# KexinZhangResearch/PhysDock

Hardware: AMD Instinct MI355X
Metric: poses/sec (whole node) at crop_size=256, atom_crop_size=2048 (higher is better)
Workload: dtype f32 (fp16x2-split operands x3 MFMA / bf16x3-split x6 MFMA, fp32 accumulate)

## Files before the change

physdock_amd/csrc/gemm_f16.hip:

```cpp
#include <stdlib.h>
#include <type_traits>
#define PD_EPILOGUE_Y2 1
#include "gemm_tile_common.h"

namespace {

typedef _Float16 f16x8 __attribute__((ext_vector_type(8)));
typedef _Float16 f16x4 __attribute__((ext_vector_type(4)));
typedef unsigned u32x2 __attribute__((ext_vector_type(2)));

constexpr int F16_MIN_TILES = 256, F16_MIN_TILES_SMALL = 160, F16_MIN_TILES_SMALL_LONGK = 96;
#ifdef PD_LAB
__device__ unsigned long long* g_f16_trace = nullptr;
#define PD_TRACE_F16_PTR g_f16_trace
#else
#define PD_TRACE_F16_PTR ((unsigned long long*)nullptr)
#endif
constexpr int NPARTS = 2;
constexpr int PITCH = 24;
constexpr int PITCH2 = 40;

template <int BM_, int BN_, int WM_, int NWAVES_, bool DW_>
struct FTile {
    static constexpr int BM = BM_, BN = BN_, WM = WM_, WN = NWAVES_ / WM_, NT = 64 * NWAVES_;
    static constexpr int TM = BM / (32 * WM), TN = BN / (32 * WN);
    static constexpr bool DW = DW_;
    static constexpr int STAGE = DW ? NPARTS * BM * PITCH2 : NPARTS * (BM + BN) * PITCH;
    static constexpr int LDS_BYTES = 2 * STAGE * 2;
    static constexpr int BLOCKS_PER_CU = NWAVES_ == 8 ? 2 : 4;
    static constexpr int WAVES_PER_SIMD = NWAVES_ * BLOCKS_PER_CU / 4;
    static constexpr int GRID = 256 * BLOCKS_PER_CU;
};

__device__ __forceinline__ void lds_barrier() {
    asm volatile("" ::: "memory");
    __builtin_amdgcn_s_waitcnt(0xc07f);
    __builtin_amdgcn_s_barrier();
    asm volatile("" ::: "memory");
}

__device__ __forceinline__ void split4h(const f32x4& v, f16x4& h, f16x4& l) {
    const pd_parts2 p0 = pd_split2h(v[0], v[1]), p1 = pd_split2h(v[2], v[3]);
    h = __builtin_bit_cast(f16x4, (u32x2){p0.h, p1.h});
    l = __builtin_bit_cast(f16x4, (u32x2){p0.l, p1.l});
}

template <int PRO, int EPI, class TL>
__global__ __launch_bounds__(TL::NT) __attribute__((amdgpu_waves_per_eu(TL::WAVES_PER_SIMD, TL::WAVES_PER_SIMD)))
void gemm_f16_kernel(const pd_gemm_args p) {
    constexpr int BM = TL::BM, BN = TL::BN, TM = TL::TM, TN = TL::TN;
    constexpr int XSLOTS = TL::GRID / 8;
    constexpr int SNT = TL::NT;
    constexpr int TPR_A = SNT / BM;
    constexpr int CPH_A = 4 / TPR_A;
    constexpr int TPR_W = SNT / BN;
    constexpr int NW = 4 / TPR_W;
    constexpr bool DW = TL::DW;
    extern __shared__ __attribute__((aligned(16))) _Float16 lds[];
    const int tid = threadIdx.x, lane = tid & 63;
    const int wave = __builtin_amdgcn_readfirstlane(tid >> 6);
    const int wm = wave / TL::WN, wn = wave % TL::WN;
    const int l31 = lane & 31, hh = lane >> 5;
    const int nMb = p.M / BM, nNb = p.N / BN;
    const int ntiles = nMb * nNb;
    const int nk = (p.K + 31) / 32;
    const int nks = 2 * nk;
    const f16x8* __restrict__ W2 = reinterpret_cast<const f16x8*>(p.W2);
    const long long wpart = (long long)((p.N + 31) / 32) * nks * 64;
    auto w2_chunk = [&](int part, int n, int kchunk) {
        return W2 + part * wpart + ((long long)(n >> 5) * nks + (kchunk >> 1)) * 64 + (kchunk & 1) * 32 + (n & 31);
    };
    const float a_s = pd_pow2_scale(*p.a_amax);
    const float inv_a_s = 1.0f / a_s;

    auto sA = [&](int s, int part) { return lds + s * TL::STAGE + part * BM * PITCH; };
    auto sW = [&](int s, int part) { return lds + s * TL::STAGE + NPARTS * BM * PITCH + part * BN * PITCH; };

    const int a_row = tid / TPR_A, a_q = tid % TPR_A;
    const int w_row = tid / TPR_W, w_q = tid % TPR_W;
    constexpr bool AS = PRO == 3;
    constexpr int CPA = 4 / TPR_A;
    const _Float16* __restrict__ A2 = reinterpret_cast<const _Float16*>(p.A2);
    const long long apart = (long long)p.M * (nk * 32);
    f16x8 ra2[NPARTS][AS ? CPA : 1];
    f32x4 ra[2][CPH_A];
    f16x8 rw[NPARTS][NW];

    auto gload = [&](int bm0, int bn0, int k0) {
        const int r = bm0 + a_row;
        if constexpr (AS) {
            const _Float16* ap2 = A2 + (long long)r * (nk * 32) + k0 + 8 * a_q;
#pragma unroll
            for (int part = 0; part < NPARTS; ++part)
#pragma unroll
                for (int i = 0; i < CPA; ++i) ra2[part][i] = *reinterpret_cast<const f16x8*>(ap2 + part * apart + 8 * TPR_A * i);
        }
        const float* ap = p.A + (long long)r * p.lda + k0;
#pragma unroll
        for (int h = 0; h < (AS ? 0 : 2); ++h)
#pragma unroll
            for (int i = 0; i < CPH_A; ++i) {
                int kc = 16 * h + 4 * (a_q + TPR_A * i);
                kc = k0 + kc < p.K ? kc : 0;
                ra[h][i] = *reinterpret_cast<const f32x4*>(ap + kc);
            }
        if constexpr (!DW) {
#pragma unroll
            for (int part = 0; part < NPARTS; ++part)
#pragma unroll
                for (int i = 0; i < NW; ++i)
                    rw[part][i] = *w2_chunk(part, bn0 + w_row, (k0 >> 3) + (NW == 2 ? w_q + 2 * i : w_q));
        }
    };
    f16x8 wf[2][TN][NPARTS];
    auto wfrag = [&](int buf, int bn0, int ks) {
#pragma unroll
        for (int j = 0; j < TN; ++j) {
            const f16x8* base = W2 + ((long long)((bn0 + wn * (32 * TN) + j * 32) >> 5) * nks + ks) * 64 + lane;
#pragma unroll
            for (int part = 0; part < NPARTS; ++part) wf[buf][j][part] = base[part * wpart];
        }
    };

    f32x16 acc[TM][TN];
    const bool grouped = gridDim.x == TL::GRID && nMb >= 8;
    TileOrder ord;
    ord.init(nMb, nNb, grouped ? blockIdx.x & 7 : 0, grouped ? 8 : 1, XSLOTS);
    const int t_step = grouped ? XSLOTS : gridDim.x;
    const int t_end = grouped ? ord.ntiles : ntiles;
    int tile = grouped ? blockIdx.x >> 3 : blockIdx.x;
    if (tile >= t_end) return;
    auto coords = [&](int t, int& bm0, int& bn0) {
        int mb, nb;
        if (grouped) ord.get(t, mb, nb);
        else { mb = t % nMb; nb = t / nMb; }
        bm0 = mb * BM; bn0 = nb * BN;
    };
    int bm0, bn0;
    coords(tile, bm0, bn0);
    gload(bm0, bn0, 0);
    if constexpr (DW) { wfrag(0, bn0, 0); wfrag(1, bn0, 1); }

    for (; tile < t_end; tile += t_step) {
        const int n0 = bn0 + wn * (32 * TN) + l31;
        float c0[TN], c1[TN], cs[TN];
        const int gate_row = bm0 + wm * (32 * TM);
#pragma unroll
        for (int j = 0; j < TN; ++j) {
            c0[j] = p.bias ? p.bias[n0 + 32 * j] : 0.f;
            c1[j] = 1.f;
            cs[j] = p.w_inv[n0 + 32 * j] * inv_a_s;
            if constexpr (EPI == EPI_HN) c1[j] = p.hn_w[((n0 + 32 * j) / p.hn_split) * 32 + l31];
            if constexpr (EPI == EPI_GATERES)
                c1[j] = p.mul ? p.mul[(long long)(gate_row / p.mul_rows_per_group) * p.mul_gstride + n0 + 32 * j] : 1.f;
        }
        float st_mean = 0.f, st_rstd = 1.f;
        int grp_off = 0;
        if constexpr (PRO != 0 && !AS) {
            const int m = bm0 + a_row;
            st_mean = p.stats[2 * (long long)m];
            st_rstd = p.stats[2 * (long long)m + 1];
            if constexpr (PRO == 2) grp_off = (m / p.pro_rows_per_group) * p.pro_gstride;
        }
        auto prep = [&](f32x4 v, int kc, f16x4& ph, f16x4& pl) {
            if constexpr (PRO != 0) {
                const int kl = kc < p.K ? kc : 0;
                const f32x4 pw = *reinterpret_cast<const f32x4*>(p.pro_w + grp_off + kl);
                const f32x4 pb = *reinterpret_cast<const f32x4*>(p.pro_b + grp_off + kl);
#pragma unroll
                for (int e = 0; e < 4; ++e) v[e] = (v[e] - st_mean) * st_rstd * pw[e] + pb[e];
            }
            if (p.pro_act == PD_ACT_RELU) {
#pragma unroll
                for (int e = 0; e < 4; ++e) v[e] = fmaxf(v[e], 0.f);
            } else if (p.pro_act == PD_ACT_SILU) {
#pragma unroll
                for (int e = 0; e < 4; ++e) v[e] = pd_silu(v[e]);
            }
#pragma unroll
            for (int e = 0; e < 4; ++e) v[e] *= a_s;
            if (kc >= p.K) v = f32x4{0.f, 0.f, 0.f, 0.f};
            split4h(v, ph, pl);
        };
        auto stage = [&](int h, int k0) {
            if constexpr (AS) {
                if ((a_q >> 1) == h) {
#pragma unroll
                    for (int part = 0; part < NPARTS; ++part)
                        *reinterpret_cast<f16x8*>(sA(h, part) + a_row * PITCH + 8 * (a_q & 1)) = ra2[part][0];
                }
            }
#pragma unroll
            for (int i = 0; i < (AS ? 0 : CPH_A); ++i) {
                const int c = a_q + TPR_A * i;
                f16x4 ph, pl;
                prep(ra[h][i], k0 + 16 * h + 4 * c, ph, pl);
                const int o = a_row * PITCH + 4 * c;
                *reinterpret_cast<f16x4*>(sA(h, 0) + o) = ph;
                *reinterpret_cast<f16x4*>(sA(h, 1) + o) = pl;
            }
            if (!DW && (NW == 2 || (w_q >> 1) == h)) {
                const int i = NW == 2 ? h : 0;
                const int c = NW == 2 ? w_q : (w_q & 1);
#pragma unroll
                for (int part = 0; part < NPARTS; ++part)
                    *reinterpret_cast<f16x8*>(sW(h, part) + w_row * PITCH + 8 * c) = rw[part][i];
            }
        };
        auto mma = [&](int s) {
            f16x8 fa[TM][NPARTS], fw[TN][NPARTS];
#pragma unroll
            for (int part = 0; part < NPARTS; ++part) {
#pragma unroll
                for (int i = 0; i < TM; ++i)
                    fa[i][part] = *reinterpret_cast<const f16x8*>(sA(s, part) + (wm * (32 * TM) + i * 32 + l31) * PITCH + 8 * hh);
#pragma unroll
                for (int j = 0; j < TN; ++j)
                    fw[j][part] = *reinterpret_cast<const f16x8*>(sW(s, part) + (wn * (32 * TN) + j * 32 + l31) * PITCH + 8 * hh);
            }
#pragma unroll
            for (int i = 0; i < TM; ++i)
#pragma unroll
                for (int j = 0; j < TN; ++j) {
                    f32x16 c = acc[i][j];
                    c = __builtin_amdgcn_mfma_f32_32x32x16_f16(fa[i][0], fw[j][1], c, 0, 0, 0);
                    c = __builtin_amdgcn_mfma_f32_32x32x16_f16(fa[i][1], fw[j][0], c, 0, 0, 0);
                    c = __builtin_amdgcn_mfma_f32_32x32x16_f16(fa[i][0], fw[j][0], c, 0, 0, 0);
                    acc[i][j] = c;
                }
        };
        auto stage2 = [&](int s, int k0) {
            _Float16* base = lds + s * TL::STAGE + a_row * PITCH2;
            if constexpr (AS) {
#pragma unroll
                for (int part = 0; part < NPARTS; ++part)
#pragma unroll
                    for (int i = 0; i < CPA; ++i) *reinterpret_cast<f16x8*>(base + part * BM * PITCH2 + 8 * (a_q + TPR_A * i)) = ra2[part][i];
            }
#pragma unroll
            for (int h = 0; h < (AS ? 0 : 2); ++h)
#pragma unroll
                for (int i = 0; i < CPH_A; ++i) {
                    const int c = a_q + TPR_A * i;
                    f16x4 ph, pl;
                    prep(ra[h][i], k0 + 16 * h + 4 * c, ph, pl);
                    const int o = 16 * h + 4 * c;
                    *reinterpret_cast<f16x4*>(base + o) = ph;
                    *reinterpret_cast<f16x4*>(base + BM * PITCH2 + o) = pl;
                }
        };
        auto mma2 = [&](int s, int ks) {
            f16x8 fa[TM][NPARTS];
            const _Float16* base = lds + s * TL::STAGE + (wm * (32 * TM) + l31) * PITCH2 + 16 * ks + 8 * hh;
#pragma unroll
            for (int part = 0; part < NPARTS; ++part)
#pragma unroll
                for (int i = 0; i < TM; ++i)
                    fa[i][part] = *reinterpret_cast<const f16x8*>(base + part * BM * PITCH2 + i * 32 * PITCH2);
#pragma unroll
            for (int i = 0; i < TM; ++i)
#pragma unroll
                for (int j = 0; j < TN; ++j) {
                    f32x16 c = acc[i][j];
                    c = __builtin_amdgcn_mfma_f32_32x32x16_f16(fa[i][0], wf[ks][j][1], c, 0, 0, 0);
                    c = __builtin_amdgcn_mfma_f32_32x32x16_f16(fa[i][1], wf[ks][j][0], c, 0, 0, 0);
                    c = __builtin_amdgcn_mfma_f32_32x32x16_f16(fa[i][0], wf[ks][j][0], c, 0, 0, 0);
                    acc[i][j] = c;
                }
        };
#pragma unroll
        for (int i = 0; i < TM; ++i)
#pragma unroll
            for (int j = 0; j < TN; ++j)
#pragma unroll
                for (int r = 0; r < 16; ++r) acc[i][j][r] = 0.f;

        lds_barrier();
        if constexpr (DW) {
            unsigned long long* dbg = nullptr;
            if (PD_TRACE_F16_PTR && lane == 0 && blockIdx.x < 64 && tile < t_step)
                dbg = PD_TRACE_F16_PTR + ((long long)blockIdx.x * 8 + wave) * (6 * 64);
#define PD_STAMP(slot) if (dbg && kt < 64) dbg[kt * 6 + slot] = __builtin_amdgcn_s_memtime()
            stage2(0, 0);
            lds_barrier();
            auto slice = [&](int kt, auto more_c) {
                constexpr bool more = decltype(more_c)::value;
                const int st = kt & 1;
                PD_STAMP(0);
                if constexpr (more) { gload(bm0, bn0, (kt + 1) * 32); __builtin_amdgcn_sched_barrier(0); }
                mma2(st, 0);
                PD_STAMP(1);
                if constexpr (more) { __builtin_amdgcn_sched_barrier(0); wfrag(0, bn0, 2 * kt + 2); __builtin_amdgcn_sched_barrier(0); }
                mma2(st, 1);
                PD_STAMP(2);
                if constexpr (more) {
                    __builtin_amdgcn_sched_barrier(0);
                    wfrag(1, bn0, 2 * kt + 3);
                    __builtin_amdgcn_sched_barrier(0);
                    PD_STAMP(3);
                    stage2(st ^ 1, (kt + 1) * 32);
                    PD_STAMP(4);
                    lds_barrier();
                    PD_STAMP(5);
                }
            };
            for (int kt = 0; kt + 1 < nk; ++kt) slice(kt, std::true_type{});
            slice(nk - 1, std::false_type{});
#undef PD_STAMP
        } else {
            stage(0, 0);
            stage(1, 0);
            lds_barrier();
            for (int kt = 0; kt < nk; ++kt) {
                const bool more = kt + 1 < nk;
                if (more) gload(bm0, bn0, (kt + 1) * 32);
                mma(0);
                if (nk > 1) lds_barrier();
                if (more) stage(0, (kt + 1) * 32);
                mma(1);
                if (more) {
                    lds_barrier();
                    stage(1, (kt + 1) * 32);
                }
            }
        }
        const int cur_bm0 = bm0, cur_bn0 = bn0;
        if (tile + t_step < t_end) {
            coords(tile + t_step, bm0, bn0);
            gload(bm0, bn0, 0);
            if constexpr (DW) { wfrag(0, bn0, 0); wfrag(1, bn0, 1); }
        }
#pragma unroll
        for (int i = 0; i < TM; ++i)
#pragma unroll
            for (int j = 0; j < TN; ++j)
#pragma unroll
                for (int r = 0; r < 16; ++r) acc[i][j][r] *= cs[j];
        epilogue<EPI, TM, TN>(p, acc, c0, c1, cur_bm0, cur_bn0, wm, wn, l31, hh);
    }
}

#ifdef PD_LAB
}
extern "C" __attribute__((visibility("default"))) int pd_lab_set_f16_trace(void* buf) {
    unsigned long long* q = reinterpret_cast<unsigned long long*>(buf);
    return hipMemcpyToSymbol(HIP_SYMBOL(g_f16_trace), &q, sizeof(q)) == hipSuccess ? PD_OK : PD_ERR_LAUNCH;
}
namespace {
#endif

template <int PRO, int EPI, class TL>
int run_f16(int op, const pd_gemm_args* p, hipStream_t s) {
    auto k = gemm_f16_kernel<PRO, EPI, TL>;
    constexpr int lds = TL::LDS_BYTES;
    if (op == 1)
        return hipFuncSetAttribute(reinterpret_cast<const void*>(k), hipFuncAttributeMaxDynamicSharedMemorySize, lds) == hipSuccess
                   ? PD_OK : PD_ERR_LAUNCH;
    const long long ntiles = (long long)(p->M / TL::BM) * (p->N / TL::BN);
    hipLaunchKernelGGL(k, dim3((unsigned)(ntiles < TL::GRID ? ntiles : TL::GRID)), dim3(TL::NT), lds, s, *p);
    return pd_check_launch();
}


constexpr int RLP = 136;
template <int PRO, int EPI, int BM>
__global__ __launch_bounds__(4 * BM) __attribute__((amdgpu_waves_per_eu(4, 4)))
void gemm_f16_rows_kernel(const pd_gemm_args p) {
    constexpr int TM = 2, TN = 1, PART = BM * RLP, NKS = 8, PF = 3, KC = 128;
    constexpr bool XPF = true;
    static_assert(NKS % (PF + 1) == 0, "the fragment ring must be back at buffer 0 when a column tile ends");
    extern __shared__ __attribute__((aligned(16))) _Float16 lds[];
    const int tid = threadIdx.x, lane = tid & 63;
    const int wave = __builtin_amdgcn_readfirstlane(tid >> 6);
    const int wm = wave >> 2, wn = wave & 3;
    const int l31 = lane & 31, hh = lane >> 5;
    const float a_s = pd_pow2_scale(*p.a_amax);
    const float inv_a_s = 1.0f / a_s;
    const int ntiles = p.M / BM, nNb = p.N / 128;
    const int wpart = (p.N >> 5) * NKS * 1024;
    const auto rs_w = __builtin_amdgcn_make_buffer_rsrc(const_cast<void*>(p.W2), 0, 2 * wpart, 0x00020000);
    const int loff = lane * 16;

    for (int tile = blockIdx.x; tile < ntiles; tile += gridDim.x) {
        const int row0 = tile * BM;
        {
            const int r = tid >> 2, q = tid & 3;
            const int m = row0 + r;
            const float* xr = p.A + (long long)m * p.lda;
            const int goff = PRO == 2 ? (m / p.pro_rows_per_group) * p.pro_gstride : 0;
            f32x4 v[8];
            float s1 = 0.f;
#pragma unroll
            for (int i = 0; i < 8; ++i) {
                v[i] = *reinterpret_cast<const f32x4*>(xr + 4 * (q + 4 * i));
                s1 += v[i][0] + v[i][1] + v[i][2] + v[i][3];
            }
            s1 += __shfl_xor(s1, 1);
            s1 += __shfl_xor(s1, 2);
            float mean = p.stats_inline == 2 ? s1 * (1.0f / KC) : 0.f;
            float sq = 0.f;
#pragma unroll
            for (int i = 0; i < 8; ++i)
#pragma unroll
                for (int e = 0; e < 4; ++e) { const float d = v[i][e] - mean; sq += d * d; }
            sq += __shfl_xor(sq, 1);
            sq += __shfl_xor(sq, 2);
            float rstd = rsqrtf(sq * (1.0f / KC) + p.stats_eps) * a_s;
            if (p.stats) {
                mean = p.stats[2 * (long long)m];
                rstd = p.stats[2 * (long long)m + 1] * a_s;
            }
#pragma unroll
            for (int i = 0; i < 8; ++i) {
                const int c = 4 * (q + 4 * i);
                const f32x4 gw = *reinterpret_cast<const f32x4*>(p.pro_w + goff + c), gb = *reinterpret_cast<const f32x4*>(p.pro_b + goff + c);
                float t[4];
#pragma unroll
                for (int e = 0; e < 4; ++e) t[e] = (v[i][e] - mean) * rstd * gw[e] + gb[e] * a_s;
                const pd_parts2 p0 = pd_split2h(t[0], t[1]), p1 = pd_split2h(t[2], t[3]);
                *reinterpret_cast<u32x2*>(lds + r * RLP + c) = u32x2{p0.h, p1.h};
                *reinterpret_cast<u32x2*>(lds + PART + r * RLP + c) = u32x2{p0.l, p1.l};
            }
        }
        lds_barrier();
        const _Float16* abase = lds + (64 * wm + l31) * RLP + 8 * hh;
        f16x8 wf[PF + 1][NPARTS];
        auto wload = [&](int cb, int buf, int ks) {
            const int so = (cb * NKS + ks) * 1024;
            wf[buf][0] = __builtin_bit_cast(f16x8, __builtin_amdgcn_raw_buffer_load_b128(rs_w, loff, so, 0));
            wf[buf][1] = __builtin_bit_cast(f16x8, __builtin_amdgcn_raw_buffer_load_b128(rs_w, loff, so + wpart, 0));
        };
#pragma unroll
        for (int ks = 0; ks < PF; ++ks) wload(wn, ks, ks);
#pragma unroll 1
        for (int nt = 0; nt < nNb; ++nt) {
            const int bn0 = nt * 128;
            const int cb = (bn0 >> 5) + wn;
            if (!XPF && nt > 0) {
#pragma unroll
                for (int ks = 0; ks < PF; ++ks) wload(cb, ks, ks);
            }
            const int n0 = bn0 + wn * 32 + l31;
            float c0[TN], c1[TN];
            c0[0] = p.bias ? p.bias[n0] : 0.f;
            c1[0] = 1.f;
            if constexpr (EPI == EPI_HN) c1[0] = p.hn_w[(n0 / p.hn_split) * 32 + l31];
            const float cs = p.w_inv[n0] * inv_a_s;
            f32x16 acc[TM][TN];
#pragma unroll
            for (int i = 0; i < TM; ++i)
#pragma unroll
                for (int r = 0; r < 16; ++r) acc[i][0][r] = 0.f;
#pragma unroll
            for (int ks = 0; ks < NKS; ++ks) {
                if (ks + PF < NKS) wload(cb, (ks + PF) % (PF + 1), ks + PF);
                __builtin_amdgcn_sched_barrier(0);
#pragma unroll
                for (int i = 0; i < TM; ++i) {
                    const f16x8 a0 = *reinterpret_cast<const f16x8*>(abase + 32 * i * RLP + 16 * ks);
                    const f16x8 a1 = *reinterpret_cast<const f16x8*>(abase + PART + 32 * i * RLP + 16 * ks);
                    f32x16 t = acc[i][0];
                    t = __builtin_amdgcn_mfma_f32_32x32x16_f16(a0, wf[ks % (PF + 1)][1], t, 0, 0, 0);
                    t = __builtin_amdgcn_mfma_f32_32x32x16_f16(a1, wf[ks % (PF + 1)][0], t, 0, 0, 0);
                    t = __builtin_amdgcn_mfma_f32_32x32x16_f16(a0, wf[ks % (PF + 1)][0], t, 0, 0, 0);
                    acc[i][0] = t;
                }
            }
            if (XPF && nt + 1 < nNb) {
#pragma unroll
                for (int ks = 0; ks < PF; ++ks) wload(cb + 4, ks, ks);
                __builtin_amdgcn_sched_barrier(0);
            }
#pragma unroll
            for (int i = 0; i < TM; ++i)
#pragma unroll
                for (int r = 0; r < 16; ++r) acc[i][0][r] *= cs;
            epilogue<EPI, TM, TN>(p, acc, c0, c1, row0, bn0, wm, wn, l31, hh);
        }
        lds_barrier();
    }
}


constexpr int WLP = 520;
constexpr int WROWS_LDS_BYTES = 2 * 64 * WLP * 2;

template <int PRO, int EPI, int TM, int TN, int GK = 4, int NWV = 16>
__global__ __launch_bounds__(64 * NWV) __attribute__((amdgpu_waves_per_eu(NWV / 4, 4)))
void gemm_f16_wrows_kernel(const pd_gemm_args p) {
    constexpr int BM = 64, KC = 512, PART = BM * WLP, NKS = KC / 16, PF = GK - 1, RG = 2 / TM;
    constexpr int RPP = 4 * NWV;
    static_assert(NKS % (PF + 1) == 0, "the fragment ring must be back at buffer 0 when a work item ends");
    static_assert(TM * RG == 2 && NWV % RG == 0, "a wave keeps its row group");
    extern __shared__ __attribute__((aligned(16))) _Float16 lds[];
    const int tid = threadIdx.x, lane = tid & 63;
    const int wave = __builtin_amdgcn_readfirstlane(tid >> 6);
    const int l31 = lane & 31, hh = lane >> 5;
    const float a_s = pd_pow2_scale(*p.a_amax);
    const float inv_a_s = 1.0f / a_s;
    const int ntiles = p.M / BM, ncb = p.N >> 5;
    const int nitems = RG * (ncb / TN);
    const int wpart = ncb * NKS * 1024;
    const auto rs_w = __builtin_amdgcn_make_buffer_rsrc(const_cast<void*>(p.W2), 0, 2 * wpart, 0x00020000);
    const int loff = lane * 16;
    const int rh = wave % RG;

    const int nsplit = (int)gridDim.x > ntiles ? (int)gridDim.x / ntiles : 1;
    for (int work = blockIdx.x; work < ntiles * nsplit; work += gridDim.x) {
        const int tile = work / nsplit, part = work - tile * nsplit;
        const int item0 = part * nitems / nsplit, item1 = (part + 1) * nitems / nsplit;
        const int row0 = tile * BM;
        if constexpr (PRO == 3) {
            const int q = tid & 15;
#pragma unroll 1
            for (int r = tid >> 4; r < BM; r += RPP) {
            const _Float16* a2 = reinterpret_cast<const _Float16*>(p.A2) + (long long)(row0 + r) * KC;
            f16x8 c[NPARTS][4];
#pragma unroll
            for (int part = 0; part < NPARTS; ++part)
#pragma unroll
                for (int i = 0; i < 4; ++i) c[part][i] = *reinterpret_cast<const f16x8*>(a2 + (long long)part * p.M * KC + 8 * (q + 16 * i));
#pragma unroll
            for (int part = 0; part < NPARTS; ++part)
#pragma unroll
                for (int i = 0; i < 4; ++i) *reinterpret_cast<f16x8*>(lds + part * PART + r * WLP + 8 * (q + 16 * i)) = c[part][i];
            }
        } else if constexpr (PRO == 0) {
            const int q = tid & 15;
#pragma unroll 1
            for (int r = tid >> 4; r < BM; r += RPP) {
                const float* xr = p.A + (long long)(row0 + r) * p.lda;
#pragma unroll
                for (int i = 0; i < 8; ++i) {
                    const int c = 4 * (q + 16 * i);
                    const f32x4 v = *reinterpret_cast<const f32x4*>(xr + c);
                    const pd_parts2 p0 = pd_split2h(v[0] * a_s, v[1] * a_s), p1 = pd_split2h(v[2] * a_s, v[3] * a_s);
                    *reinterpret_cast<u32x2*>(lds + r * WLP + c) = u32x2{p0.h, p1.h};
                    *reinterpret_cast<u32x2*>(lds + PART + r * WLP + c) = u32x2{p0.l, p1.l};
                }
            }
        } else {
            const int q = tid & 15;
#pragma unroll 1
            for (int r = tid >> 4; r < BM; r += RPP) {
            const int m = row0 + r;
            const float* xr = p.A + (long long)m * p.lda;
            const int goff = PRO == 2 ? (m / p.pro_rows_per_group) * p.pro_gstride : 0;
            f32x4 v[8];
            float s1 = 0.f;
#pragma unroll
            for (int i = 0; i < 8; ++i) {
                v[i] = *reinterpret_cast<const f32x4*>(xr + 4 * (q + 16 * i));
                s1 += v[i][0] + v[i][1] + v[i][2] + v[i][3];
            }
            auto row16 = [](float x) {
                x += pd_dpp<0xB1>(x); x += pd_dpp<0x4E>(x); x += pd_dpp<0x141>(x); x += pd_dpp<0x140>(x);
                return x;
            };
            s1 = row16(s1);
            float mean = p.stats_inline == 2 ? s1 * (1.0f / KC) : 0.f;
            float sq = 0.f;
#pragma unroll
            for (int i = 0; i < 8; ++i)
#pragma unroll
                for (int e = 0; e < 4; ++e) { const float d = v[i][e] - mean; sq += d * d; }
            sq = row16(sq);
            float rstd = rsqrtf(sq * (1.0f / KC) + p.stats_eps) * a_s;
            if (p.stats) {
                mean = p.stats[2 * (long long)m];
                rstd = p.stats[2 * (long long)m + 1] * a_s;
            }
#pragma unroll
            for (int i = 0; i < 8; ++i) {
                const int c = 4 * (q + 16 * i);
                const f32x4 gw = *reinterpret_cast<const f32x4*>(p.pro_w + goff + c), gb = *reinterpret_cast<const f32x4*>(p.pro_b + goff + c);
                float t[4];
#pragma unroll
                for (int e = 0; e < 4; ++e) t[e] = (v[i][e] - mean) * rstd * gw[e] + gb[e] * a_s;
                const pd_parts2 p0 = pd_split2h(t[0], t[1]), p1 = pd_split2h(t[2], t[3]);
                *reinterpret_cast<u32x2*>(lds + r * WLP + c) = u32x2{p0.h, p1.h};
                *reinterpret_cast<u32x2*>(lds + PART + r * WLP + c) = u32x2{p0.l, p1.l};
            }
            }
        }
        lds_barrier();
        const _Float16* abase = lds + (32 * TM * rh + l31) * WLP + 8 * hh;
        f16x8 wf[PF + 1][TN][NPARTS];
        auto wload = [&](int cu, int buf, int ks) {
#pragma unroll
            for (int j = 0; j < TN; ++j) {
                const int so = ((cu * TN + j) * NKS + ks) * 1024;
                wf[buf][j][0] = __builtin_bit_cast(f16x8, __builtin_amdgcn_raw_buffer_load_b128(rs_w, loff, so, 0));
                wf[buf][j][1] = __builtin_bit_cast(f16x8, __builtin_amdgcn_raw_buffer_load_b128(rs_w, loff, so + wpart, 0));
            }
        };
        if (item0 + wave < item1) {
#pragma unroll
            for (int ks = 0; ks < PF; ++ks) wload((item0 + wave) / RG, ks, ks);
        }
#pragma unroll 1
        for (int item = item0 + wave; item < item1; item += NWV) {
            const int cu = item / RG;
            const int n0 = cu * (32 * TN) + l31;
            float c0[TN], c1[TN], cs[TN];
#pragma unroll
            for (int j = 0; j < TN; ++j) {
                c0[j] = p.bias ? p.bias[n0 + 32 * j] : 0.f;
                c1[j] = 1.f;
                if constexpr (EPI == EPI_HN) c1[j] = p.hn_w[((n0 + 32 * j) / p.hn_split) * 32 + l31];
                if constexpr (EPI == EPI_GATERES)
                    c1[j] = p.mul ? p.mul[(long long)((row0 + 32 * TM * rh) / p.mul_rows_per_group) * p.mul_gstride + n0 + 32 * j] : 1.f;
                cs[j] = p.w_inv[n0 + 32 * j] * inv_a_s;
            }
            f32x16 acc[TM][TN];
#pragma unroll
            for (int i = 0; i < TM; ++i)
#pragma unroll
                for (int j = 0; j < TN; ++j)
#pragma unroll
                    for (int r = 0; r < 16; ++r) acc[i][j][r] = 0.f;
            auto group = [&](int ks0, auto last_c) {
                constexpr bool last = decltype(last_c)::value;
#pragma unroll
                for (int jj = 0; jj < PF + 1; ++jj) {
                    const int ks = ks0 + jj;
                    if constexpr (!last) wload(cu, (jj + PF) % (PF + 1), ks + PF);
                    else if (jj == 0) wload(cu, PF % (PF + 1), ks + PF);
                    else if (item + NWV < item1) wload((item + NWV) / RG, (jj + PF) % (PF + 1), jj - 1);
                    __builtin_amdgcn_sched_barrier(0);
#pragma unroll
                    for (int i = 0; i < TM; ++i) {
                        const f16x8 a0 = *reinterpret_cast<const f16x8*>(abase + 32 * i * WLP + 16 * ks);
                        const f16x8 a1 = *reinterpret_cast<const f16x8*>(abase + PART + 32 * i * WLP + 16 * ks);
#pragma unroll
                        for (int j = 0; j < TN; ++j) {
                            f32x16 t = acc[i][j];
                            t = __builtin_amdgcn_mfma_f32_32x32x16_f16(a0, wf[jj][j][1], t, 0, 0, 0);
                            t = __builtin_amdgcn_mfma_f32_32x32x16_f16(a1, wf[jj][j][0], t, 0, 0, 0);
                            t = __builtin_amdgcn_mfma_f32_32x32x16_f16(a0, wf[jj][j][0], t, 0, 0, 0);
                            acc[i][j] = t;
                        }
                    }
                }
            };
#pragma unroll 1
            for (int ks0 = 0; ks0 < NKS - (PF + 1); ks0 += PF + 1) group(ks0, std::false_type{});
            group(NKS - (PF + 1), std::true_type{});
#pragma unroll
            for (int i = 0; i < TM; ++i)
#pragma unroll
                for (int j = 0; j < TN; ++j)
#pragma unroll
                    for (int r = 0; r < 16; ++r) acc[i][j][r] *= cs[j];
            epilogue<EPI, TM, TN>(p, acc, c0, c1, row0, cu * (32 * TN), rh, 0, l31, hh);
        }
        lds_barrier();
    }
}


constexpr int F16_WROWS_MAX_SPLIT = 4, F16_WROWS_MIN_ITEMS = 8;
template <int PRO, int EPI, int TM, int TN, int GK = 4, int NWV = 16>
int run_f16_wrows(int op, const pd_gemm_args* p, hipStream_t s) {
    auto k = gemm_f16_wrows_kernel<PRO, EPI, TM, TN, GK, NWV>;
    if (op == 1)
        return hipFuncSetAttribute(reinterpret_cast<const void*>(k), hipFuncAttributeMaxDynamicSharedMemorySize, WROWS_LDS_BYTES) == hipSuccess
                   ? PD_OK : PD_ERR_LAUNCH;
    const int ntiles = p->M / 64;
    const int nitems = (2 / TM) * ((p->N >> 5) / TN);
    const bool few = ntiles < 32;
    int nsplit = (PRO != 3 && ntiles < 256) ? 256 / ntiles : 1;
    const int max_split = few ? 4 * F16_WROWS_MAX_SPLIT : F16_WROWS_MAX_SPLIT;
    nsplit = nsplit > max_split ? max_split : nsplit;
    while (nsplit > 1 && nitems / nsplit < (few ? F16_WROWS_MIN_ITEMS / 4 : F16_WROWS_MIN_ITEMS)) --nsplit;
    if (PRO != 3 && ntiles > 128 && ntiles < 256) {
        float best = 1e9f;
        for (int sp = 1; sp <= 6 && nitems / sp >= F16_WROWS_MIN_ITEMS; ++sp) {
            const float c = (float)((ntiles * sp + 255) / 256) * (0.15f + 1.0f / (float)sp);
            if (c < best - 1e-4f) { best = c; nsplit = sp; }
        }
    }
    hipLaunchKernelGGL(k, dim3((unsigned)(nsplit > 1 ? ntiles * nsplit : (ntiles < 256 ? ntiles : 256))), dim3(64 * NWV), WROWS_LDS_BYTES, s, *p);
    return pd_check_launch();
}

int dispatch_f16_wrows(int op, int pro, int epi, const pd_gemm_args* p, hipStream_t s) {
    if (pro == 1 && epi == EPI_HN) return run_f16_wrows<1, EPI_HN, 2, 1>(op, p, s);
    if (pro == 2 && epi == EPI_HN) return run_f16_wrows<2, EPI_HN, 2, 1>(op, p, s);
    if (pro == 1 && epi == EPI_PLAIN) return run_f16_wrows<1, EPI_PLAIN, 2, 1>(op, p, s);
    if (pro == 2 && epi == EPI_PLAIN) return run_f16_wrows<2, EPI_PLAIN, 2, 1>(op, p, s);
    if (pro == 3 && epi == EPI_GATERES) return run_f16_wrows<3, EPI_GATERES, 2, 1>(op, p, s);
    if (pro == 3 && epi == EPI_PLAIN) return run_f16_wrows<3, EPI_PLAIN, 2, 1>(op, p, s);
    if (pro == 0 && epi == EPI_GATERES) return run_f16_wrows<0, EPI_GATERES, 2, 1>(op, p, s);
    if (pro == 0 && epi == EPI_PLAIN) return run_f16_wrows<0, EPI_PLAIN, 2, 1>(op, p, s);
    if (pro == 1 && epi == EPI_GLU) return run_f16_wrows<1, EPI_GLU, 2, 2, 2>(op, p, s);
    if (pro == 2 && epi == EPI_GLU) return run_f16_wrows<2, EPI_GLU, 2, 2, 2>(op, p, s);

    return PD_ERR_UNSUPPORTED;
}


constexpr int CLP = 264;
constexpr int WCHUNK_LDS_BYTES = 2 * 2 * 64 * CLP * 2;

template <int EPI>
__global__ __launch_bounds__(1024) __attribute__((amdgpu_waves_per_eu(4, 4)))
void gemm_f16_wchunk_kernel(const pd_gemm_args p) {
    constexpr int BM = 64, KCH = 256, TM = 2, TN = 1, PART = BM * CLP, BUF = NPARTS * PART, PF = 3, GK = PF + 1;
    extern __shared__ __attribute__((aligned(16))) _Float16 lds[];
    const int tid = threadIdx.x, lane = tid & 63;
    const int wave = __builtin_amdgcn_readfirstlane(tid >> 6);
    const int l31 = lane & 31, hh = lane >> 5;
    const float a_s = pd_pow2_scale(*p.a_amax);
    const float inv_a_s = 1.0f / a_s;
    const int ntiles = p.M / BM;
    const int nks = p.K >> 4;
    const int nch = (p.K + KCH - 1) / KCH;
    const int wpart = (p.N >> 5) * nks * 1024;
    const auto rs_w = __builtin_amdgcn_make_buffer_rsrc(const_cast<void*>(p.W2), 0, 2 * wpart, 0x00020000);
    const int loff = lane * 16;
    const int sr = tid >> 4, sq = tid & 15;

    for (int tile = blockIdx.x; tile < ntiles; tile += gridDim.x) {
        const int row0 = tile * BM;
        const float* xr = p.A + (long long)(row0 + sr) * p.lda;
        f32x4 ra[4];
        auto gload = [&](int c) {
#pragma unroll
            for (int i = 0; i < 4; ++i) {
                const int col = KCH * c + 4 * (sq + 16 * i);
                ra[i] = col < p.K ? *reinterpret_cast<const f32x4*>(xr + col) : f32x4{0.f, 0.f, 0.f, 0.f};
            }
        };
        auto sstore = [&](int buf) {
            _Float16* base = lds + buf * BUF + sr * CLP;
#pragma unroll
            for (int i = 0; i < 4; ++i) {
                const int c = 4 * (sq + 16 * i);
                const pd_parts2 p0 = pd_split2h(ra[i][0] * a_s, ra[i][1] * a_s), p1 = pd_split2h(ra[i][2] * a_s, ra[i][3] * a_s);
                *reinterpret_cast<u32x2*>(base + c) = u32x2{p0.h, p1.h};
                *reinterpret_cast<u32x2*>(base + PART + c) = u32x2{p0.l, p1.l};
            }
        };
        f16x8 wf[GK][NPARTS];
        auto wload = [&](int buf, int ks) {
            const int so = (wave * nks + ks) * 1024;
            wf[buf][0] = __builtin_bit_cast(f16x8, __builtin_amdgcn_raw_buffer_load_b128(rs_w, loff, so, 0));
            wf[buf][1] = __builtin_bit_cast(f16x8, __builtin_amdgcn_raw_buffer_load_b128(rs_w, loff, so + wpart, 0));
        };
        gload(0);
#pragma unroll
        for (int ks = 0; ks < PF; ++ks) wload(ks, ks);
        const int n0 = wave * 32 + l31;
        float c0[TN], c1[TN];
        c0[0] = p.bias ? p.bias[n0] : 0.f;
        c1[0] = 1.f;
        if constexpr (EPI == EPI_GATERES) c1[0] = p.mul ? p.mul[(long long)(row0 / p.mul_rows_per_group) * p.mul_gstride + n0] : 1.f;
        const float cs = p.w_inv[n0] * inv_a_s;
        f32x16 acc[TM][TN];
#pragma unroll
        for (int i = 0; i < TM; ++i)
#pragma unroll
            for (int r = 0; r < 16; ++r) acc[i][0][r] = 0.f;
        sstore(0);
        lds_barrier();
#pragma unroll 1
        for (int c = 0; c < nch; ++c) {
            gload(c + 1);
            __builtin_amdgcn_sched_barrier(0);
            const _Float16* abase = lds + (c & 1) * BUF + l31 * CLP + 8 * hh;
            const int ng = (c + 1 < nch ? KCH / 16 : nks - c * (KCH / 16)) / GK;
#pragma unroll 1
            for (int gi = 0; gi < ng; ++gi) {
                const int ksl = gi * GK, ksg = c * (KCH / 16) + ksl;
#pragma unroll
                for (int jj = 0; jj < GK; ++jj) {
                    wload((jj + PF) % GK, ksg + jj + PF);
                    __builtin_amdgcn_sched_barrier(0);
#pragma unroll
                    for (int i = 0; i < TM; ++i) {
                        const f16x8 a0 = *reinterpret_cast<const f16x8*>(abase + 32 * i * CLP + 16 * (ksl + jj));
                        const f16x8 a1 = *reinterpret_cast<const f16x8*>(abase + PART + 32 * i * CLP + 16 * (ksl + jj));
                        f32x16 t = acc[i][0];
                        t = __builtin_amdgcn_mfma_f32_32x32x16_f16(a0, wf[jj][1], t, 0, 0, 0);
                        t = __builtin_amdgcn_mfma_f32_32x32x16_f16(a1, wf[jj][0], t, 0, 0, 0);
                        t = __builtin_amdgcn_mfma_f32_32x32x16_f16(a0, wf[jj][0], t, 0, 0, 0);
                        acc[i][0] = t;
                    }
                }
            }
            if (c + 1 < nch) sstore((c + 1) & 1);
            lds_barrier();
        }
#pragma unroll
        for (int i = 0; i < TM; ++i)
#pragma unroll
            for (int r = 0; r < 16; ++r) acc[i][0][r] *= cs;
        epilogue<EPI, TM, TN>(p, acc, c0, c1, row0, wave * 32, 0, 0, l31, hh);
    }
}

template <int EPI>
int run_f16_wchunk(int op, const pd_gemm_args* p, hipStream_t s) {
    auto k = gemm_f16_wchunk_kernel<EPI>;
    if (op == 1)
        return hipFuncSetAttribute(reinterpret_cast<const void*>(k), hipFuncAttributeMaxDynamicSharedMemorySize, WCHUNK_LDS_BYTES) == hipSuccess
                   ? PD_OK : PD_ERR_LAUNCH;
    const int ntiles = p->M / 64;
    hipLaunchKernelGGL(k, dim3((unsigned)(ntiles < 256 ? ntiles : 256)), dim3(1024), WCHUNK_LDS_BYTES, s, *p);
    return pd_check_launch();
}

int dispatch_f16_wchunk(int op, int epi, const pd_gemm_args* p, hipStream_t s) {
    if (epi == EPI_GATERES) return run_f16_wchunk<EPI_GATERES>(op, p, s);
    if (epi == EPI_PLAIN) return run_f16_wchunk<EPI_PLAIN>(op, p, s);
    return PD_ERR_UNSUPPORTED;
}

constexpr int F16_WROWS_PLAIN_MAX_TILES = 39;
constexpr int F16_WROWS_MIN_TILES_SPLIT = 4;
constexpr int F16_WROWS_MIN_TILES = 128;

template <int PRO, int EPI, int BM>
int run_f16_rows(int op, const pd_gemm_args* p, hipStream_t s) {
    auto k = gemm_f16_rows_kernel<PRO, EPI, BM>;
    constexpr int lds = 2 * BM * RLP * 2;
    if (op == 1)
        return hipFuncSetAttribute(reinterpret_cast<const void*>(k), hipFuncAttributeMaxDynamicSharedMemorySize, lds) == hipSuccess
                   ? PD_OK : PD_ERR_LAUNCH;
    const int ntiles = p->M / BM, grid = 512 * (128 / BM);
    hipLaunchKernelGGL(k, dim3((unsigned)(ntiles < grid ? ntiles : grid)), dim3(4 * BM), lds, s, *p);
    return pd_check_launch();
}

int dispatch_f16_rows(int op, int pro, int epi, const pd_gemm_args* p, hipStream_t s, bool big) {
#define PD_RCASE(P, E) if (pro == P && epi == E) { \
        if (op == 1) { const int r = run_f16_rows<P, E, 64>(1, p, s); return r != PD_OK ? r : run_f16_rows<P, E, 128>(1, p, s); } \
        return big ? run_f16_rows<P, E, 128>(op, p, s) : run_f16_rows<P, E, 64>(op, p, s); }
    PD_RCASE(1, EPI_HN) PD_RCASE(2, EPI_HN) PD_RCASE(1, EPI_PLAIN) PD_RCASE(2, EPI_PLAIN)
#undef PD_RCASE
    return PD_ERR_UNSUPPORTED;
}

constexpr int F16_ROWS_MIN_TILES = 512;
constexpr int F16_ROWS_MIN_TILES64 = 320;

using F128 = FTile<128, 128, 2, 8, true>;
using F128G = FTile<128, 128, 4, 8, false>;
using F128GD = FTile<128, 128, 4, 8, true>;

using F64 = FTile<64, 128, 1, 4, true>;

int dispatch_f16(int op, int pro, int epi, const pd_gemm_args* p, hipStream_t s, bool small) {
#define PD_FCASE(P, E, TL) if (pro == P && epi == E) return run_f16<P, E, TL>(op, p, s);
    if (small) {
        PD_FCASE(0, EPI_PLAIN, F64) PD_FCASE(1, EPI_PLAIN, F64) PD_FCASE(3, EPI_PLAIN, F64)
        PD_FCASE(1, EPI_HN, F64) PD_FCASE(2, EPI_HN, F64) PD_FCASE(3, EPI_HN, F64)
        PD_FCASE(0, EPI_GATERES, F64) PD_FCASE(3, EPI_GATERES, F64) PD_FCASE(0, EPI_TGATERES, F64)
        return PD_ERR_UNSUPPORTED;
    }
    PD_FCASE(0, EPI_PLAIN, F128) PD_FCASE(1, EPI_PLAIN, F128) PD_FCASE(3, EPI_PLAIN, F128)
    PD_FCASE(1, EPI_HN, F128) PD_FCASE(2, EPI_HN, F128) PD_FCASE(3, EPI_HN, F128)
    PD_FCASE(1, EPI_GLU, F128G) PD_FCASE(2, EPI_GLU, F128G) PD_FCASE(3, EPI_GLU, F128GD) PD_FCASE(1, EPI_GLUT, F128G)
    PD_FCASE(0, EPI_GATERES, F128) PD_FCASE(3, EPI_GATERES, F128) PD_FCASE(0, EPI_TGATERES, F128)
#undef PD_FCASE
    return PD_ERR_UNSUPPORTED;
}

}

extern "C" int pd_gemm_f16_try(const pd_gemm_args* args, int pro, int tile, void* stream, int init_only) {
    if (init_only == 1) {
        int rc = PD_OK;
        for (int P = 0; P < 4; ++P)
            for (int E = 0; E < 6; ++E) {
                for (int small = 0; small < 2; ++small) {
                    const int r = dispatch_f16(1, P, E, nullptr, nullptr, small != 0);
                    if (r != PD_OK && r != PD_ERR_UNSUPPORTED) rc = r;
                }
                const int r = dispatch_f16_rows(1, P, E, nullptr, nullptr, true);
                if (r != PD_OK && r != PD_ERR_UNSUPPORTED) rc = r;
                const int rw = dispatch_f16_wrows(1, P, E, nullptr, nullptr);
                if (rw != PD_OK && rw != PD_ERR_UNSUPPORTED) rc = rw;
                const int rc2 = P == 0 ? dispatch_f16_wchunk(1, E, nullptr, nullptr) : PD_ERR_UNSUPPORTED;
                if (rc2 != PD_OK && rc2 != PD_ERR_UNSUPPORTED) rc = rc2;
            }
        return rc;
    }
    const pd_gemm_args& p = *args;
    if (!p.W2 || !p.w_inv || !p.a_amax || p.K % 4 != 0 || (tile != 128 && tile != 64)) return PD_ERR_UNSUPPORTED;
    if (p.A2) {
        if (pro != 0 || p.pro_act != PD_ACT_NONE || p.K % 32 != 0 || ((uintptr_t)p.A2 & 15)) return PD_ERR_UNSUPPORTED;
        pro = 3;
    }
    const bool glut = p.out_mode == PD_OUT_TRANSPOSED && p.glu && !p.hn_w && !p.mul && !p.res && !p.act && !p.rowscale_acc &&
                      !p.maskadd && p.out_scale == 1.f && p.vecY && (!p.rowscale || ((uintptr_t)p.rowscale & 15) == 0) && !p.A2 && !p.Y2;
    if (p.a_kmajor || p.w_kmajor || !p.vecA || p.batch != 1 || (p.out_mode != PD_OUT_ROWMAJOR && !glut)) return PD_ERR_UNSUPPORTED;
    if (((uintptr_t)p.W2 & 15) != 0 || p.N % 128 != 0 || p.M % 64 != 0) return PD_ERR_UNSUPPORTED;
    const long long t128 = p.M % 128 == 0 ? (long long)(p.M / 128) * (p.N / 128) : 0, t64 = (long long)(p.M / 64) * (p.N / 128);
    const bool tiny = t128 < F16_MIN_TILES && t64 < (p.K >= 1024 ? F16_MIN_TILES_SMALL_LONGK : F16_MIN_TILES_SMALL);
    const bool plain512 = p.K == 512 && !p.A2 && pro == 0 && !p.stats && !p.stats_inline && p.pro_act == PD_ACT_NONE &&
                          p.M / 64 >= F16_WROWS_MIN_TILES_SPLIT && p.M / 64 <= F16_WROWS_PLAIN_MAX_TILES && t128 < F16_MIN_TILES;
    if (tiny && !(p.K == 512 && !p.A2 && !p.stats && (p.stats_inline || plain512))) return PD_ERR_UNSUPPORTED;
    const bool small = t128 < F16_MIN_TILES;
    if (p.rowscale_acc || (p.rowscale && !glut) || p.maskadd || p.out_scale != 1.f) return PD_ERR_UNSUPPORTED;
    int epi;
    if (glut) epi = small ? -1 : EPI_GLUT;
    else if (p.glu) epi = (p.hn_w || p.mul || p.res || p.act) ? -1 : EPI_GLU;
    else if (p.hn_w) epi = (p.mul || p.res || p.act) ? -1 : EPI_HN;
    else if (p.res) {
        epi = (p.mul && p.mul_rows_per_group <= 0) ? EPI_TGATERES : EPI_GATERES;
        if (p.act || p.res_row_mod > 0) epi = -1;
        if (p.mul && p.mul_rows_per_group > 0 && p.mul_rows_per_group % 64 != 0) epi = -1;
    } else epi = p.mul ? -1 : EPI_PLAIN;
    if (epi < 0) return PD_ERR_UNSUPPORTED;
    if (p.Y2) {
        if (epi != EPI_HN || !p.y2_amax || p.hn_split <= 0 || p.hn_split % 32 != 0 || p.y2_col0 % 32 != 0 ||
            p.ldy2 < 2 * (p.N - p.y2_col0) || p.ldy2 % 8 != 0 || ((uintptr_t)p.Y2 & 15))
            return PD_ERR_UNSUPPORTED;
    }
    const bool rows_big = p.M % 128 == 0 && p.M / 128 >= F16_ROWS_MIN_TILES;
    const bool rows_ok = p.K == 128 && !p.A2 && (pro == 1 || pro == 2) && p.pro_act == PD_ACT_NONE && p.act == PD_ACT_NONE &&
                         (rows_big || p.M / 64 >= F16_ROWS_MIN_TILES64) && (epi == EPI_HN || epi == EPI_PLAIN) &&
                         (p.stats || p.stats_inline == 1 || p.stats_inline == 2) && p.lda % 4 == 0 && ((uintptr_t)p.A & 15) == 0 &&
                         (((uintptr_t)p.pro_w | (uintptr_t)p.pro_b) & 15) == 0 && p.pro_gstride % 4 == 0 &&
                         (pro != 2 || p.pro_rows_per_group > 0) && (long long)(p.N / 32) * 8 * 1024 * 2 < 0x7fffffffll;
    const bool wrows_ok = p.K == 512 && !p.A2 && !p.stats && (pro == 1 || pro == 2) && p.pro_act == PD_ACT_NONE && p.act == PD_ACT_NONE &&
                          p.M % 64 == 0 && p.M / 64 >= F16_WROWS_MIN_TILES_SPLIT && (epi == EPI_HN || epi == EPI_PLAIN || (epi == EPI_GLU && p.N % 64 == 0)) &&
                          (p.stats_inline == 1 || p.stats_inline == 2) && p.lda % 4 == 0 && ((uintptr_t)p.A & 15) == 0 &&
                          (((uintptr_t)p.pro_w | (uintptr_t)p.pro_b) & 15) == 0 && p.pro_gstride % 4 == 0 &&
                          (pro != 2 || p.pro_rows_per_group > 0) && (long long)(p.N / 32) * 32 * 1024 * 2 < 0x7fffffffll;
    const bool wrows_a2 = p.K == 512 && p.A2 && pro == 3 && p.act == PD_ACT_NONE && p.M / 64 >= F16_WROWS_MIN_TILES && p.M % 64 == 0 &&
                          (epi == EPI_PLAIN || (epi == EPI_GATERES && (!p.mul || p.mul_rows_per_group % 64 == 0))) &&
                          (long long)(p.N / 32) * 32 * 1024 * 2 < 0x7fffffffll;
    const bool wchunk_ok = p.N == 512 && p.K > 512 && p.K % 64 == 0 && !p.A2 && !p.stats && !p.stats_inline && pro == 0 &&
                           p.pro_act == PD_ACT_NONE && p.act == PD_ACT_NONE && p.M % 64 == 0 && p.M / 64 >= F16_WROWS_MIN_TILES &&
                           p.lda % 4 == 0 && ((uintptr_t)p.A & 15) == 0 &&
                           (epi == EPI_PLAIN || (epi == EPI_GATERES && (!p.mul || p.mul_rows_per_group % 64 == 0))) &&
                           (long long)16 * (p.K / 16) * 1024 * 2 < 0x7fffffffll;
    if (wchunk_ok) {
        if (init_only == 2) {
            const int r = dispatch_f16_wchunk(1, epi, nullptr, nullptr);
            return r == PD_OK ? epi + 0x600 : r;
        }
        return dispatch_f16_wchunk(0, epi, &p, (hipStream_t)stream);
    }
    const bool wrows_plain = plain512 && p.act == PD_ACT_NONE && p.M % 64 == 0 && p.lda % 4 == 0 && ((uintptr_t)p.A & 15) == 0 &&
                             (epi == EPI_PLAIN || (epi == EPI_GATERES && (!p.mul || p.mul_rows_per_group % 64 == 0))) &&
                             (long long)(p.N / 32) * 32 * 1024 * 2 < 0x7fffffffll;
    if (wrows_ok || wrows_a2 || wrows_plain) {
        if (init_only == 2) {
            const int r = dispatch_f16_wrows(1, pro, epi, nullptr, nullptr);
            return r == PD_OK ? epi + 0x500 : r;
        }
        return dispatch_f16_wrows(0, pro, epi, &p, (hipStream_t)stream);
    }
    if (tiny) return PD_ERR_UNSUPPORTED;
    if ((!p.stats && p.stats_inline) || rows_ok) {
        const bool big = rows_big;
        if (!rows_ok) return PD_ERR_UNSUPPORTED;
        if (init_only == 2) {
            const int r = dispatch_f16_rows(1, pro, epi, nullptr, nullptr, big);
            return r == PD_OK ? epi + (big ? 0x300 : 0x400) : r;
        }
        return dispatch_f16_rows(0, pro, epi, &p, (hipStream_t)stream, big);
    }
    if (init_only == 2) {
        const int r = dispatch_f16(1, pro, epi, nullptr, nullptr, small);
        return r == PD_OK ? epi + (small ? 0x100 : 0) : r;
    }
    return dispatch_f16(0, pro, epi, &p, (hipStream_t)stream, small);
}
```

Baseline: 164.8.

## Swap MFMA operands in HN rows kernel for row-per-lane epilogue

For the head-norm epilogue in the K=128 rows kernel, the MFMA operands are swapped so each lane holds a row's columns instead of a column's rows. A new epilogue uses this transposed accumulator layout to apply per-column scale, bias and head-norm weights with vector loads, compute the per-row sum of squares mostly in-lane, and write outputs as vector stores. It aims to cut cross-lane reductions and scalar stores in the epilogue. In exchange it adds alignment and hn_split preconditions that can send some cases to other kernels, and per-row behaviour now depends on a new helper reduction.

```diff
diff --git a/physdock_amd/csrc/gemm_f16.hip b/physdock_amd/csrc/gemm_f16.hip
--- a/physdock_amd/csrc/gemm_f16.hip
+++ b/physdock_amd/csrc/gemm_f16.hip
@@ -8,6 +8,7 @@
 typedef _Float16 f16x8 __attribute__((ext_vector_type(8)));
 typedef _Float16 f16x4 __attribute__((ext_vector_type(4)));
 typedef unsigned u32x2 __attribute__((ext_vector_type(2)));
+typedef unsigned u32x4 __attribute__((ext_vector_type(4)));
 
 constexpr int F16_MIN_TILES = 256, F16_MIN_TILES_SMALL = 160, F16_MIN_TILES_SMALL_LONGK = 96;
 #ifdef PD_LAB
@@ -43,6 +44,100 @@
     const pd_parts2 p0 = pd_split2h(v[0], v[1]), p1 = pd_split2h(v[2], v[3]);
     h = __builtin_bit_cast(f16x4, (u32x2){p0.h, p1.h});
     l = __builtin_bit_cast(f16x4, (u32x2){p0.l, p1.l});
+}
+
+template <bool XCH>
+__device__ __forceinline__ f32x16 mfma3(const f16x8& a0, const f16x8& a1, const f16x8& w0, const f16x8& w1, f32x16 c) {
+    if constexpr (XCH) {
+        c = __builtin_amdgcn_mfma_f32_32x32x16_f16(w1, a0, c, 0, 0, 0);
+        c = __builtin_amdgcn_mfma_f32_32x32x16_f16(w0, a1, c, 0, 0, 0);
+        c = __builtin_amdgcn_mfma_f32_32x32x16_f16(w0, a0, c, 0, 0, 0);
+    } else {
+        c = __builtin_amdgcn_mfma_f32_32x32x16_f16(a0, w1, c, 0, 0, 0);
+        c = __builtin_amdgcn_mfma_f32_32x32x16_f16(a1, w0, c, 0, 0, 0);
+        c = __builtin_amdgcn_mfma_f32_32x32x16_f16(a0, w0, c, 0, 0, 0);
+    }
+    return c;
+}
+
+template <int TM>
+__device__ __forceinline__ void epilogue_hn_rowlane(const pd_gemm_args& p, f32x16 (&acc)[TM][1], float inv_a_s, int mb0, int ncol0,
+                                                    int l31, int hh) {
+#pragma clang fp contract(off)
+    asm volatile("" : "+v"(l31), "+v"(hh));
+    const bool normed = ncol0 < p.hn_cols;
+    const bool to_y2 = p.Y2 != nullptr && ncol0 >= p.y2_col0;
+    float ss[TM];
+    f32x4 bv[4];
+#pragma unroll
+    for (int i = 0; i < TM; ++i) ss[i] = 0.f;
+#pragma unroll
+    for (int g = 0; g < 4; ++g) bv[g] = f32x4{0.f, 0.f, 0.f, 0.f};
+    if (p.bias) {
+#pragma unroll
+        for (int g = 0; g < 4; ++g) bv[g] = *reinterpret_cast<const f32x4*>(p.bias + ncol0 + 8 * g + 4 * hh);
+    }
+#pragma unroll
+    for (int g = 0; g < 4; ++g) {
+        const f32x4 wi = *reinterpret_cast<const f32x4*>(p.w_inv + ncol0 + 8 * g + 4 * hh);
+#pragma unroll
+        for (int e = 0; e < 4; ++e) {
+            const float cs = wi[e] * inv_a_s;
+#pragma unroll
+            for (int i = 0; i < TM; ++i) {
+                const float v = acc[i][0][4 * g + e] * cs + bv[g][e];
+                acc[i][0][4 * g + e] = v;
+                ss[i] = __builtin_fmaf(v, v, ss[i]);
+            }
+        }
+    }
+    float rs[TM];
+    f32x4 hw[4];
+    if (normed) {
+        const float* __restrict__ hwp = p.hn_w + (ncol0 / p.hn_split) * 32;
+#pragma unroll
+        for (int g = 0; g < 4; ++g) hw[g] = *reinterpret_cast<const f32x4*>(hwp + 8 * g + 4 * hh);
+#pragma unroll
+        for (int i = 0; i < TM; ++i) rs[i] = rsqrtf(pd_xhalf_sum(ss[i]) * (1.0f / 32.0f) + p.hn_eps);
+    } else {
+#pragma unroll
+        for (int g = 0; g < 4; ++g) hw[g] = f32x4{1.f, 1.f, 1.f, 1.f};
+#pragma unroll
+        for (int i = 0; i < TM; ++i) rs[i] = 1.f;
+    }
+    if (to_y2) {
+        const float y2s = pd_pow2_scale(p.y2_amax[(ncol0 - p.y2_col0) / p.hn_split]);
+        _Float16* __restrict__ Y2o = reinterpret_cast<_Float16*>(p.Y2) + (long long)mb0 * p.ldy2 + 2 * (ncol0 - p.y2_col0);
+        const int y2off = l31 * p.ldy2 + 8 * hh;
+#pragma unroll
+        for (int i = 0; i < TM; ++i)
+#pragma unroll
+            for (int g = 0; g < 4; ++g) {
+                float o[4];
+#pragma unroll
+                for (int e = 0; e < 4; ++e) {
+                    const float v = acc[i][0][4 * g + e];
+                    o[e] = (normed ? v * rs[i] * hw[g][e] : v) * y2s;
+                }
+                const pd_parts2 p0 = pd_split2h(o[0], o[1]), p1 = pd_split2h(o[2], o[3]);
+                *reinterpret_cast<u32x4*>(Y2o + (32 * i) * p.ldy2 + 16 * g + y2off) = u32x4{p0.h, p1.h, p0.l, p1.l};
+            }
+    } else {
+        float* __restrict__ Yo = p.Y + (long long)mb0 * p.ldy + ncol0;
+        const int yoff = l31 * p.ldy + 4 * hh;
+#pragma unroll
+        for (int i = 0; i < TM; ++i)
+#pragma unroll
+            for (int g = 0; g < 4; ++g) {
+                f32x4 o;
+#pragma unroll
+                for (int e = 0; e < 4; ++e) {
+                    const float v = acc[i][0][4 * g + e];
+                    o[e] = normed ? v * rs[i] * hw[g][e] : v;
+                }
+                *reinterpret_cast<f32x4*>(Yo + (32 * i) * p.ldy + 8 * g + yoff) = o;
+            }
+    }
 }
 
 template <int PRO, int EPI, class TL>
@@ -367,6 +462,7 @@
 __global__ __launch_bounds__(4 * BM) __attribute__((amdgpu_waves_per_eu(4, 4)))
 void gemm_f16_rows_kernel(const pd_gemm_args p) {
     constexpr int TM = 2, TN = 1, PART = BM * RLP, NKS = 8, PF = 3, KC = 128;
+    constexpr bool XCH = EPI == EPI_HN;
     constexpr bool XPF = true;
     static_assert(NKS % (PF + 1) == 0, "the fragment ring must be back at buffer 0 when a column tile ends");
     extern __shared__ __attribute__((aligned(16))) _Float16 lds[];
@@ -444,7 +540,6 @@
             float c0[TN], c1[TN];
             c0[0] = p.bias ? p.bias[n0] : 0.f;
             c1[0] = 1.f;
-            if constexpr (EPI == EPI_HN) c1[0] = p.hn_w[(n0 / p.hn_split) * 32 + l31];
             const float cs = p.w_inv[n0] * inv_a_s;
             f32x16 acc[TM][TN];
 #pragma unroll
@@ -459,11 +554,7 @@
                 for (int i = 0; i < TM; ++i) {
                     const f16x8 a0 = *reinterpret_cast<const f16x8*>(abase + 32 * i * RLP + 16 * ks);
                     const f16x8 a1 = *reinterpret_cast<const f16x8*>(abase + PART + 32 * i * RLP + 16 * ks);
-                    f32x16 t = acc[i][0];
-                    t = __builtin_amdgcn_mfma_f32_32x32x16_f16(a0, wf[ks % (PF + 1)][1], t, 0, 0, 0);
-                    t = __builtin_amdgcn_mfma_f32_32x32x16_f16(a1, wf[ks % (PF + 1)][0], t, 0, 0, 0);
-                    t = __builtin_amdgcn_mfma_f32_32x32x16_f16(a0, wf[ks % (PF + 1)][0], t, 0, 0, 0);
-                    acc[i][0] = t;
+                    acc[i][0] = mfma3<XCH>(a0, a1, wf[ks % (PF + 1)][0], wf[ks % (PF + 1)][1], acc[i][0]);
                 }
             }
             if (XPF && nt + 1 < nNb) {
@@ -471,11 +562,15 @@
                 for (int ks = 0; ks < PF; ++ks) wload(cb + 4, ks, ks);
                 __builtin_amdgcn_sched_barrier(0);
             }
-#pragma unroll
-            for (int i = 0; i < TM; ++i)
-#pragma unroll
-                for (int r = 0; r < 16; ++r) acc[i][0][r] *= cs;
-            epilogue<EPI, TM, TN>(p, acc, c0, c1, row0, bn0, wm, wn, l31, hh);
+            if constexpr (XCH) {
+                epilogue_hn_rowlane<TM>(p, acc, inv_a_s, row0 + 64 * wm, bn0 + wn * 32, l31, hh);
+            } else {
+#pragma unroll
+                for (int i = 0; i < TM; ++i)
+#pragma unroll
+                    for (int r = 0; r < 16; ++r) acc[i][0][r] *= cs;
+                epilogue<EPI, TM, TN>(p, acc, c0, c1, row0, bn0, wm, wn, l31, hh);
+            }
         }
         lds_barrier();
     }
@@ -924,7 +1019,9 @@
                          (rows_big || p.M / 64 >= F16_ROWS_MIN_TILES64) && (epi == EPI_HN || epi == EPI_PLAIN) &&
                          (p.stats || p.stats_inline == 1 || p.stats_inline == 2) && p.lda % 4 == 0 && ((uintptr_t)p.A & 15) == 0 &&
                          (((uintptr_t)p.pro_w | (uintptr_t)p.pro_b) & 15) == 0 && p.pro_gstride % 4 == 0 &&
-                         (pro != 2 || p.pro_rows_per_group > 0) && (long long)(p.N / 32) * 8 * 1024 * 2 < 0x7fffffffll;
+                         (pro != 2 || p.pro_rows_per_group > 0) && (long long)(p.N / 32) * 8 * 1024 * 2 < 0x7fffffffll &&
+                         (epi != EPI_HN || (p.hn_split > 0 && p.hn_split % 32 == 0 && p.ldy % 4 == 0 &&
+                                            (((uintptr_t)p.Y | (uintptr_t)p.hn_w | (uintptr_t)p.w_inv | (uintptr_t)p.bias) & 15) == 0));
     const bool wrows_ok = p.K == 512 && !p.A2 && !p.stats && (pro == 1 || pro == 2) && p.pro_act == PD_ACT_NONE && p.act == PD_ACT_NONE &&
                           p.M % 64 == 0 && p.M / 64 >= F16_WROWS_MIN_TILES_SPLIT && (epi == EPI_HN || epi == EPI_PLAIN || (epi == EPI_GLU && p.N % 64 == 0)) &&
                           (p.stats_inline == 1 || p.stats_inline == 2) && p.lda % 4 == 0 && ((uintptr_t)p.A & 15) == 0 &&
```

After: 164.9 (median of 4 runs). No clear change (+0.1%).
